# OpenBMB/VisRAG

Measured on NVIDIA H100. Metric: page-images encoded/sec, higher is better.
Workload: dtype bf16

## Files before the change

### visrag_b200/csrc/gemm.cu

```cuda
#include "common.h"
#include "gemm.cuh"

namespace vr {

template <bool F16, int BN, int MODE, bool OUT_F32, bool GELU, bool SWAP = false>
static int launch_gemm(const void* A, int64_t lda, const void* B, int64_t ldb, const GemmArgs& g, cudaStream_t stream) {
    using Cfg = GemmCfg<BN>;
    CUtensorMap ta, tb;
    if (int rc = make_tmap_2d(SWAP ? &tb : &ta, A, g.M, g.K, lda, SWAP ? 64 : GEMM_BM, GEMM_BK, 128, !F16)) return rc;
    if (int rc = make_tmap_2d(SWAP ? &ta : &tb, B, g.N, g.K, ldb, SWAP ? GEMM_BM : 64, GEMM_BK, 128, !F16)) return rc;
    auto kern = gemm_wgmma_kernel<F16, BN, MODE, OUT_F32, GELU, SWAP>;
    static unsigned long long attr_set = 0;
    if (first_use_on_device(&attr_set))
        VR_CHECK_CUDA(cudaFuncSetAttribute(kern, cudaFuncAttributeMaxDynamicSharedMemorySize, Cfg::SMEM_BYTES));
    const int tiles = SWAP ? ((g.N + GEMM_BM - 1) / GEMM_BM) * ((g.M + BN - 1) / BN)
                           : ((g.M + GEMM_BM - 1) / GEMM_BM) * ((g.N + BN - 1) / BN);
    const int grid = tiles < num_sms() ? tiles : num_sms();
    kern<<<grid, GEMM_THREADS, Cfg::SMEM_BYTES, stream>>>(ta, tb, g);
    VR_CHECK_CUDA(cudaGetLastError());
    return 0;
}

template <bool F16, int MODE, bool OUT_F32, bool GELU, int CLUSTER>
static int launch_pingpong(const void* A, int64_t lda, const void* B, int64_t ldb, const GemmArgs& g, bool l2_slices,
                           cudaStream_t stream) {
    CUtensorMap ta, tb;
    if (int rc = make_tmap_2d(&ta, A, g.M, g.K, lda, GEMM_BM, GEMM_BK, 128, !F16)) return rc;
    if (int rc = make_tmap_2d(&tb, B, g.N, g.K, ldb, 64, GEMM_BK, 128, !F16)) return rc;
    auto kern = gemm_pingpong_kernel<F16, MODE, OUT_F32, GELU, CLUSTER>;
    cudaLaunchConfig_t cfg = {};
    cudaLaunchAttribute attr[1];
    cfg.blockDim = dim3(GEMM_THREADS);
    cfg.dynamicSmemBytes = GEMM_PP_SMEM_BYTES;
    cfg.stream = stream;
    attr[0].id = cudaLaunchAttributeClusterDimension;
    attr[0].val.clusterDim.x = CLUSTER;
    attr[0].val.clusterDim.y = 1;
    attr[0].val.clusterDim.z = 1;
    cfg.attrs = attr;
    cfg.numAttrs = 1;
    static unsigned long long attr_set = 0;
    static int max_clusters[64] = {};
    const int dev = current_device(), dev_slot = dev >= 0 && dev < 64 ? dev : 0;
    if (first_use_on_device(&attr_set)) {
        VR_CHECK_CUDA(cudaFuncSetAttribute(kern, cudaFuncAttributeMaxDynamicSharedMemorySize, GEMM_PP_SMEM_BYTES));
        int n = num_sms() / CLUSTER;
        if (CLUSTER > 1) {
            cfg.gridDim = dim3(num_sms() / CLUSTER * CLUSTER);
            VR_CHECK_CUDA(cudaOccupancyMaxActiveClusters(&n, kern, &cfg));
        }
        max_clusters[dev_slot] = n;
    }
    const PPSched sch = pp_schedule(g.M, g.N, g.K, CLUSTER, l2_slices);
    VR_REQUIRE(max_clusters[dev_slot] > 0, "vr_gemm: no %d-CTA cluster of the ping-pong kernel fits on this device", CLUSTER);
    const int units = sch.num_units();
    const int clusters = units < max_clusters[dev_slot] ? units : max_clusters[dev_slot];
    cfg.gridDim = dim3(clusters * CLUSTER);
    VR_CHECK_CUDA(cudaLaunchKernelEx(&cfg, kern, ta, tb, g, sch));
    return 0;
}

template <bool F16>
static int check_out_dtype(const vr_gemm_epilogue& e) {
    if (F16) {
        if (e.mode == VR_EPI_LINEAR && e.out_dtype == VR_F32) {
            VR_REQUIRE(!e.act_gelu, "vr_gemm: GELU epilogue writes fp16 only (fp16 operands)");
            return 0;
        }
        if (e.mode == VR_EPI_LINEAR)
            VR_REQUIRE(e.out_dtype == VR_F16, "vr_gemm: with fp16 operands out_dtype must be VR_F16 or VR_F32");
        else
            VR_REQUIRE(e.out_dtype == VR_F16, "vr_gemm: with fp16 operands ROPE / SWIGLU write fp16: out_dtype must be VR_F16");
        return 0;
    }
    if (e.mode != VR_EPI_LINEAR) return 0;
    if (e.out_dtype == VR_F32) {
        VR_REQUIRE(!e.act_gelu, "vr_gemm: GELU epilogue writes bf16 only");
        return 0;
    }
    VR_REQUIRE(e.out_dtype == VR_BF16, "vr_gemm: out_dtype must be VR_BF16 or VR_F32");
    return 0;
}

template <bool F16>
static int dispatch_swapped(const void* A, int64_t lda, const void* B, int64_t ldb, const GemmArgs& g, cudaStream_t s) {
    const vr_gemm_epilogue& e = g.epi;
    VR_REQUIRE(e.mode == VR_EPI_LINEAR, "vr_gemm: block_n=3 (feature-major accumulator) supports LINEAR epilogues only");
    if (int rc = check_out_dtype<F16>(e)) return rc;
    if (e.out_dtype == VR_F32) return launch_gemm<F16, 128, VR_EPI_LINEAR, true, false, true>(A, lda, B, ldb, g, s);
    if (e.act_gelu) return launch_gemm<F16, 128, VR_EPI_LINEAR, false, true, true>(A, lda, B, ldb, g, s);
    return launch_gemm<F16, 128, VR_EPI_LINEAR, false, false, true>(A, lda, B, ldb, g, s);
}

constexpr int PP = 2, PP_MC = 4, PP_NFAST = 5;
template <bool F16, int BN, int MODE, bool OUT_F32, bool GELU>
static int launch_any(const void* A, int64_t lda, const void* B, int64_t ldb, const GemmArgs& g, cudaStream_t s) {
    if constexpr (BN < 0) return launch_pingpong<F16, MODE, OUT_F32, GELU, -BN == PP_MC ? 2 : 1>(A, lda, B, ldb, g, -BN != PP_NFAST, s);
    else return launch_gemm<F16, BN, MODE, OUT_F32, GELU>(A, lda, B, ldb, g, s);
}

template <bool F16, int BN>
static int dispatch_mode(const void* A, int64_t lda, const void* B, int64_t ldb, const GemmArgs& g, cudaStream_t s) {
    const vr_gemm_epilogue& e = g.epi;
    switch (e.mode) {
        case VR_EPI_LINEAR:
            if (int rc = check_out_dtype<F16>(e)) return rc;
            if (e.out_dtype == VR_F32) return launch_any<F16, BN, VR_EPI_LINEAR, true, false>(A, lda, B, ldb, g, s);
            if (e.act_gelu) return launch_any<F16, BN, VR_EPI_LINEAR, false, true>(A, lda, B, ldb, g, s);
            return launch_any<F16, BN, VR_EPI_LINEAR, false, false>(A, lda, B, ldb, g, s);
        case VR_EPI_ROPE:
            VR_REQUIRE(e.positions && e.rope_cos && e.rope_sin, "vr_gemm: ROPE epilogue needs positions/cos/sin");
            VR_REQUIRE(g.N % 64 == 0 && e.rope_cols % 64 == 0, "vr_gemm: ROPE needs N and rope_cols multiples of 64");
            if (int rc = check_out_dtype<F16>(e)) return rc;
            return launch_any<F16, BN, VR_EPI_ROPE, false, false>(A, lda, B, ldb, g, s);
        case VR_EPI_SWIGLU:
            VR_REQUIRE(g.N % 64 == 0, "vr_gemm: SWIGLU needs N multiple of 64");
            if (int rc = check_out_dtype<F16>(e)) return rc;
            return launch_any<F16, BN, VR_EPI_SWIGLU, false, false>(A, lda, B, ldb, g, s);
        default:
            set_error("vr_gemm: unknown epilogue mode %d", e.mode);
            return 2;
    }
}

template <bool F16>
static int dispatch_block_n(const void* A, int64_t lda, const void* B, int64_t ldb, const GemmArgs& g, int bn, cudaStream_t s) {
    if (bn == PP) return dispatch_mode<F16, -PP>(A, lda, B, ldb, g, s);
    if (bn == PP_MC) return dispatch_mode<F16, -PP_MC>(A, lda, B, ldb, g, s);
    if (bn == PP_NFAST) return dispatch_mode<F16, -PP_NFAST>(A, lda, B, ldb, g, s);
    if (bn == 3) return dispatch_swapped<F16>(A, lda, B, ldb, g, s);
    if (bn == 256) return dispatch_mode<F16, 256>(A, lda, B, ldb, g, s);
    if (bn == 192) return dispatch_mode<F16, 192>(A, lda, B, ldb, g, s);
    if (bn == 128) return dispatch_mode<F16, 128>(A, lda, B, ldb, g, s);
    if (bn == 64) return dispatch_mode<F16, 64>(A, lda, B, ldb, g, s);
    set_error("vr_gemm: block_n must be 0 (auto), 64, 128, 192, 256, 2 / 4 / 5 (ping-pong) or 3 (feature-major accumulator)");
    return 2;
}

}

extern "C" int vr_gemm_tuned(const void* A, int64_t lda, const void* B, int64_t ldb, int32_t ab_dtype, int32_t M,
                             int32_t N, int32_t K, const vr_gemm_epilogue* epi, int32_t block_n, void* stream) {
    using namespace vr;
    VR_REQUIRE(A && B && epi && epi->out, "vr_gemm: null pointer argument");
    VR_REQUIRE(M > 0 && N > 0 && K > 0, "vr_gemm: empty problem M=%d N=%d K=%d", M, N, K);
    VR_REQUIRE(ab_dtype == VR_BF16 || ab_dtype == VR_F16, "vr_gemm: operands must be bf16 or fp16 (got dtype %d)", ab_dtype);
    VR_REQUIRE(N % 8 == 0, "vr_gemm: N=%d must be a multiple of 8", N);
    VR_REQUIRE(K % 8 == 0, "vr_gemm: K=%d must be a multiple of 8 (16-byte TMA rows)", K);
    const int64_t out_cols = epi->mode == VR_EPI_SWIGLU ? N / 2 : N;
    VR_REQUIRE(epi->ldo >= out_cols && epi->ldo % 8 == 0, "vr_gemm: ldo=%lld too small or not a multiple of 8",
               (long long)epi->ldo);
    GemmArgs g;
    g.M = M; g.N = N; g.K = K; g.epi = *epi;
    cudaStream_t s = reinterpret_cast<cudaStream_t>(stream);
    int bn = block_n;
    if (bn == 0) {
        bn = M <= 128 ? 64 : PP_MC;
    }
    return ab_dtype == VR_F16 ? dispatch_block_n<true>(A, lda, B, ldb, g, bn, s) : dispatch_block_n<false>(A, lda, B, ldb, g, bn, s);
}

extern "C" int vr_gemm(const void* A, int64_t lda, const void* B, int64_t ldb, int32_t ab_dtype, int32_t M, int32_t N,
                       int32_t K, const vr_gemm_epilogue* epi, void* stream) {
    return vr_gemm_tuned(A, lda, B, ldb, ab_dtype, M, N, K, epi, 0, stream);
}
```

### visrag_b200/csrc/gemm.cuh

```cuda
#pragma once
#include "ptx.cuh"
#include "../../include/visrag_b200.h"

namespace vr {

constexpr int GEMM_BM = 128;
constexpr int GEMM_BK = 64;
constexpr int GEMM_THREADS = 3 * 128;

template <int BN>
struct GemmCfg {
    static_assert(BN % 64 == 0 && BN <= 256, "tile width: 64, 128, 192 or 256");
    static constexpr int A_BYTES = GEMM_BM * GEMM_BK * 2;
    static constexpr int B_BYTES = BN * GEMM_BK * 2;
    static constexpr int STAGE_BYTES = A_BYTES + B_BYTES;
    static constexpr int STAGES = (192 * 1024) / STAGE_BYTES;
    static constexpr int SMEM_BYTES = STAGES * STAGE_BYTES + 1024  + 256 ;
};

struct GemmArgs {
    int M, N, K;
    vr_gemm_epilogue epi;
};

__device__ __forceinline__ float erf_as(float x) {
    const float ax = fabsf(x);
    float t;
    asm("rcp.approx.ftz.f32 %0, %1;" : "=f"(t) : "f"(fmaf(0.3275911f, ax, 1.0f)));
    float p = fmaf(1.061405429f, t, -1.453152027f);
    p = fmaf(p, t, 1.421413741f);
    p = fmaf(p, t, -0.284496736f);
    p = fmaf(p, t, 0.254829592f);
    p *= t;
    float e;
    asm("ex2.approx.ftz.f32 %0, %1;" : "=f"(e) : "f"(-1.4426950408889634f * ax * ax));
    return copysignf(fmaf(-p, e, 1.0f), x);
}
__device__ __forceinline__ float gelu_erf(float x) { return 0.5f * x * (1.0f + erf_as(x * 0.70710678118654752f)); }

__device__ __forceinline__ void pk_fma(float& d0, float& d1, float a0, float a1, float b0, float b1, float c0, float c1) {
    d0 = fmaf(a0, b0, c0);
    d1 = fmaf(a1, b1, c1);
}
#ifndef VR_GELU_POLY
#define VR_GELU_POLY 1
#endif
#if VR_GELU_POLY
__device__ __forceinline__ void gelu_erf2(float& x0, float& x1) {
    constexpr float R2 = 0.70710678118654752f, ZMAX = 3.2f, A = 2.0f / (ZMAX * ZMAX);
    const float z0 = fminf(fmaxf(x0 * R2, -ZMAX), ZMAX), z1 = fminf(fmaxf(x1 * R2, -ZMAX), ZMAX);
    float w0, w1, u0, u1, p0, p1;
    pk_fma(w0, w1, z0, z1, z0, z1, 0.0f, 0.0f);
    pk_fma(u0, u1, w0, w1, A, A, -1.0f, -1.0f);
    pk_fma(p0, p1, u0, u1, 2.982273671e-03f, 2.982273671e-03f, -7.046153472e-03f, -7.046153472e-03f);
    pk_fma(p0, p1, p0, p1, u0, u1, 7.957076705e-03f, 7.957076705e-03f);
    pk_fma(p0, p1, p0, p1, u0, u1, -1.521942819e-02f, -1.521942819e-02f);
    pk_fma(p0, p1, p0, p1, u0, u1, 3.318292224e-02f, 3.318292224e-02f);
    pk_fma(p0, p1, p0, p1, u0, u1, -5.471928813e-02f, -5.471928813e-02f);
    pk_fma(p0, p1, p0, p1, u0, u1, 8.062700147e-02f, 8.062700147e-02f);
    pk_fma(p0, p1, p0, p1, u0, u1, -1.136467381e-01f, -1.136467381e-01f);
    pk_fma(p0, p1, p0, p1, u0, u1, 1.543549678e-01f, 1.543549678e-01f);
    pk_fma(p0, p1, p0, p1, u0, u1, -2.173077339e-01f, -2.173077339e-01f);
    pk_fma(p0, p1, p0, p1, u0, u1, 4.413341836e-01f, 4.413341836e-01f);
    float r0, r1;
    pk_fma(r0, r1, p0, p1, z0, z1, 0.0f, 0.0f);
    const float h0 = 0.5f * x0, h1 = 0.5f * x1;
    pk_fma(x0, x1, h0, h1, r0, r1, h0, h1);
}
#else
__device__ __forceinline__ void gelu_erf2(float& x0, float& x1) {
    constexpr float R2 = 0.70710678118654752f;
    const float a0 = fabsf(x0) * R2, a1 = fabsf(x1) * R2;
    float d0, d1, t0, t1, p0, p1, q0, q1, e0, e1, r0, r1;
    pk_fma(d0, d1, a0, a1, 0.3275911f, 0.3275911f, 1.0f, 1.0f);
    asm("rcp.approx.ftz.f32 %0, %1;" : "=f"(t0) : "f"(d0));
    asm("rcp.approx.ftz.f32 %0, %1;" : "=f"(t1) : "f"(d1));
    pk_fma(p0, p1, t0, t1, 1.061405429f, 1.061405429f, -1.453152027f, -1.453152027f);
    pk_fma(p0, p1, p0, p1, t0, t1, 1.421413741f, 1.421413741f);
    pk_fma(p0, p1, p0, p1, t0, t1, -0.284496736f, -0.284496736f);
    pk_fma(p0, p1, p0, p1, t0, t1, 0.254829592f, 0.254829592f);
    pk_fma(p0, p1, p0, p1, t0, t1, 0.0f, 0.0f);
    pk_fma(q0, q1, a0, a1, a0, a1, 0.0f, 0.0f);
    asm("ex2.approx.ftz.f32 %0, %1;" : "=f"(e0) : "f"(q0 * -1.4426950408889634f));
    asm("ex2.approx.ftz.f32 %0, %1;" : "=f"(e1) : "f"(q1 * -1.4426950408889634f));
    pk_fma(r0, r1, p0, p1, -e0, -e1, 1.0f, 1.0f);
    r0 = copysignf(r0, x0);
    r1 = copysignf(r1, x1);
    const float h0 = 0.5f * x0, h1 = 0.5f * x1;
    pk_fma(x0, x1, h0, h1, r0, r1, h0, h1);
}
#endif
__device__ __forceinline__ float silu(float x) {
    float e, r;
    asm("ex2.approx.ftz.f32 %0, %1;" : "=f"(e) : "f"(x * -1.4426950408889634f));
    asm("rcp.approx.ftz.f32 %0, %1;" : "=f"(r) : "f"(1.0f + e));
    return x * r;
}

template <bool F16, bool OUT_F32, bool GELU>
__device__ __forceinline__ void epi_linear2(const GemmArgs& g, int row, int col, float x0, float x1) {
    const vr_gemm_epilogue& e = g.epi;
    if (row >= g.M || col >= g.N) return;
    if (e.bias) {
        const float2 b = *reinterpret_cast<const float2*>(e.bias + col);
        x0 += b.x; x1 += b.y;
    }
    if (GELU) gelu_erf2(x0, x1);
    if (e.scale != 1.0f) { x0 *= e.scale; x1 *= e.scale; }
    if (e.rowadd) {
        const float2 a2 = *reinterpret_cast<const float2*>(e.rowadd + static_cast<long long>(row % e.rowadd_period) * g.N + col);
        x0 += a2.x; x1 += a2.y;
    }
    const long long o = static_cast<long long>(row) * e.ldo + col;
    if (e.resid) {
        const float2 r2 = *reinterpret_cast<const float2*>(e.resid + o);
        x0 += r2.x; x1 += r2.y;
    }
    if (OUT_F32) *reinterpret_cast<float2*>(reinterpret_cast<float*>(e.out) + o) = make_float2(x0, x1);
    else *reinterpret_cast<uint32_t*>(reinterpret_cast<half16_t<F16>*>(e.out) + o) = pack16x2<F16>(x0, x1);
}

template <bool F16, bool OUT_F32, bool GELU>
__device__ __forceinline__ void epi_linear_t(const GemmArgs& g, int tok, int f, float x) {
    const vr_gemm_epilogue& e = g.epi;
    if (tok >= g.M || f >= g.N) return;
    if (e.bias) x += e.bias[f];
    if (GELU) {
        float y = x;
        gelu_erf2(x, y);
    }
    if (e.scale != 1.0f) x *= e.scale;
    if (e.rowadd) x += e.rowadd[static_cast<long long>(tok % e.rowadd_period) * g.N + f];
    const long long o = static_cast<long long>(tok) * e.ldo + f;
    if (e.resid) x += e.resid[o];
    if (OUT_F32) reinterpret_cast<float*>(e.out)[o] = x;
    else reinterpret_cast<half16_t<F16>*>(e.out)[o] = to_half16<F16>(x);
}

template <bool F16>
__device__ __forceinline__ void epi_rope2(const GemmArgs& g, int row, int head0, int c, float lo0, float lo1, float hi0,
                                          float hi1) {
    const vr_gemm_epilogue& e = g.epi;
    if (row >= g.M || head0 >= g.N) return;
    if (head0 < e.rope_cols) {
        const long long pos = e.positions[row];
        const float2 cs = *reinterpret_cast<const float2*>(e.rope_cos + pos * 32 + c);
        const float2 sn = *reinterpret_cast<const float2*>(e.rope_sin + pos * 32 + c);
        const float a0 = lo0, a1 = lo1, b0 = hi0, b1 = hi1;
        lo0 = a0 * cs.x - b0 * sn.x; hi0 = b0 * cs.x + a0 * sn.x;
        lo1 = a1 * cs.y - b1 * sn.y; hi1 = b1 * cs.y + a1 * sn.y;
    }
    half16_t<F16>* o = reinterpret_cast<half16_t<F16>*>(e.out) + static_cast<long long>(row) * e.ldo + head0 + c;
    *reinterpret_cast<uint32_t*>(o) = pack16x2<F16>(lo0, lo1);
    *reinterpret_cast<uint32_t*>(o + 32) = pack16x2<F16>(hi0, hi1);
}

template <bool F16>
__device__ __forceinline__ void epi_swiglu2(const GemmArgs& g, int row, int blk0, int c, float g0, float g1, float u0, float u1) {
    const vr_gemm_epilogue& e = g.epi;
    if (row >= g.M || blk0 >= g.N) return;
    half16_t<F16>* o = reinterpret_cast<half16_t<F16>*>(e.out) + static_cast<long long>(row) * e.ldo + (blk0 >> 1) + c;
    *reinterpret_cast<uint32_t*>(o) = pack16x2<F16>(silu(g0) * u0, silu(g1) * u1);
}

template <bool F16, int BN, int MODE, bool OUT_F32, bool GELU, bool SWAP = false>
__global__ void __launch_bounds__(GEMM_THREADS, 1)
gemm_wgmma_kernel(const __grid_constant__ CUtensorMap tmap_a, const __grid_constant__ CUtensorMap tmap_b, const GemmArgs g) {
    using Cfg = GemmCfg<BN>;
    constexpr int STAGES = Cfg::STAGES;

    extern __shared__ uint8_t smem_raw[];
    uint8_t* smem = reinterpret_cast<uint8_t*>((reinterpret_cast<uintptr_t>(smem_raw) + 1023) & ~uintptr_t(1023));
    uint8_t* smem_a = smem;
    uint8_t* smem_b = smem + STAGES * Cfg::A_BYTES;
    uint64_t* full_bar = reinterpret_cast<uint64_t*>(smem + STAGES * Cfg::STAGE_BYTES);
    uint64_t* empty_bar = full_bar + STAGES;

    const int wg = threadIdx.x >> 7;
    const int warp = (threadIdx.x >> 5) & 3;
    const int lane = threadIdx.x & 31;

    static_assert(!SWAP || MODE == VR_EPI_LINEAR, "feature-major accumulators are implemented for LINEAR epilogues");
    const int tiles_m = ((SWAP ? g.N : g.M) + GEMM_BM - 1) / GEMM_BM;
    const int tiles_n = ((SWAP ? g.M : g.N) + BN - 1) / BN;
    const int num_tiles = tiles_m * tiles_n;
    const int num_kb = (g.K + GEMM_BK - 1) / GEMM_BK;
    auto tile_m0 = [&](int t) { return (SWAP ? t % tiles_m : t / tiles_n) * GEMM_BM; };
    auto tile_n0 = [&](int t) { return (SWAP ? t / tiles_m : t % tiles_n) * BN; };

    if (threadIdx.x == 0) {
        tma_prefetch_desc(&tmap_a);
        tma_prefetch_desc(&tmap_b);
        for (int i = 0; i < STAGES; ++i) {
            mbar_init(&full_bar[i], 1);
            mbar_init(&empty_bar[i], 8);
        }
        fence_mbar_init();
    }
    __syncthreads();

    if (wg == 0) {
        setmaxnreg_dec<40>();
        if (warp == 0 && lane == 0) {
            int stage = 0;
            uint32_t phase = 0;
            for (int t = blockIdx.x; t < num_tiles; t += gridDim.x) {
                const int m0 = tile_m0(t);
                const int n0 = tile_n0(t);
                for (int kb = 0; kb < num_kb; ++kb) {
                    mbar_wait(&empty_bar[stage], phase ^ 1);
                    mbar_expect_tx(&full_bar[stage], Cfg::STAGE_BYTES);
                    tma_load_2d(&tmap_a, &full_bar[stage], smem_a + stage * Cfg::A_BYTES, kb * GEMM_BK, m0);
#pragma unroll
                    for (int h = 0; h < BN / 64; ++h)
                        tma_load_2d(&tmap_b, &full_bar[stage], smem_b + stage * Cfg::B_BYTES + h * (64 * GEMM_BK * 2),
                                    kb * GEMM_BK, n0 + h * 64);
                    if (++stage == STAGES) { stage = 0; phase ^= 1; }
                }
            }
        }
    } else {
        setmaxnreg_inc<232>();
        const int cw = wg - 1;
        const uint64_t desc_hi = make_smem_desc(0, 16, 1024, kLayoutSW128);
        const uint32_t a_lo0 = (smem_u32(smem_a) + cw * (64 * GEMM_BK * 2)) >> 4, b_lo0 = smem_u32(smem_b) >> 4;
        const int g8 = lane >> 2, q = lane & 3;
        int stage = 0;
        uint32_t phase = 0;
        for (int t = blockIdx.x; t < num_tiles; t += gridDim.x) {
            float acc[BN / 2];
            int prev = -1;
            for (int kb = 0; kb < num_kb; ++kb) {
                mbar_wait(&full_bar[stage], phase);
                const uint64_t ad = desc_hi | static_cast<uint64_t>(a_lo0 + stage * (Cfg::A_BYTES >> 4));
                const uint64_t bd = desc_hi | static_cast<uint64_t>(b_lo0 + stage * (Cfg::B_BYTES >> 4));
                wgmma_fence();
#pragma unroll
                for (int kk = 0; kk < 4; ++kk)
                    wgmma_ss<F16, false>(acc, ad + 2 * kk, bd + 2 * kk, (kb | kk) != 0, std::integral_constant<int, BN>());
                wgmma_commit();
                if (prev >= 0) {
                    wgmma_wait<1>();
                    if (lane == 0) mbar_arrive(&empty_bar[prev]);
                }
                prev = stage;
                if (++stage == STAGES) { stage = 0; phase ^= 1; }
            }
            wgmma_wait<0>();
            if (lane == 0) mbar_arrive(&empty_bar[prev]);
            wgmma_touch(acc);

            const int r0 = tile_m0(t) + cw * 64 + warp * 16 + g8;
            const int n0 = tile_n0(t);
            if (MODE == VR_EPI_LINEAR) {
#pragma unroll
                for (int j = 0; j < BN / 8; ++j) {
                    const int c = n0 + j * 8 + q * 2;
                    if (SWAP) {
                        epi_linear_t<F16, OUT_F32, GELU>(g, c, r0, acc[4 * j]);
                        epi_linear_t<F16, OUT_F32, GELU>(g, c + 1, r0, acc[4 * j + 1]);
                        epi_linear_t<F16, OUT_F32, GELU>(g, c, r0 + 8, acc[4 * j + 2]);
                        epi_linear_t<F16, OUT_F32, GELU>(g, c + 1, r0 + 8, acc[4 * j + 3]);
                    } else {
                        epi_linear2<F16, OUT_F32, GELU>(g, r0, c, acc[4 * j], acc[4 * j + 1]);
                        epi_linear2<F16, OUT_F32, GELU>(g, r0 + 8, c, acc[4 * j + 2], acc[4 * j + 3]);
                    }
                }
            } else {
#pragma unroll
                for (int hb = 0; hb < BN / 64; ++hb) {
#pragma unroll
                    for (int j = 0; j < 4; ++j) {
                        const int lo = 4 * (hb * 8 + j), hi = 4 * (hb * 8 + j + 4);
                        const int blk0 = n0 + hb * 64, c = j * 8 + q * 2;
                        if (MODE == VR_EPI_ROPE) {
                            epi_rope2<F16>(g, r0, blk0, c, acc[lo], acc[lo + 1], acc[hi], acc[hi + 1]);
                            epi_rope2<F16>(g, r0 + 8, blk0, c, acc[lo + 2], acc[lo + 3], acc[hi + 2], acc[hi + 3]);
                        } else {
                            epi_swiglu2<F16>(g, r0, blk0, c, acc[lo], acc[lo + 1], acc[hi], acc[hi + 1]);
                            epi_swiglu2<F16>(g, r0 + 8, blk0, c, acc[lo + 2], acc[lo + 3], acc[hi + 2], acc[hi + 3]);
                        }
                    }
                }
            }
        }
    }
}

constexpr int GEMM_PP_BN = 128;
constexpr int GEMM_PP_A_BYTES = GEMM_BM * GEMM_BK * 2;
constexpr int GEMM_PP_B_BYTES = GEMM_PP_BN * GEMM_BK * 2;
constexpr int GEMM_PP_STAGE_BYTES = GEMM_PP_A_BYTES + GEMM_PP_B_BYTES;
constexpr int GEMM_PP_STAGES = (192 * 1024) / GEMM_PP_STAGE_BYTES;
constexpr int GEMM_PP_SMEM_BYTES = GEMM_PP_STAGES * GEMM_PP_STAGE_BYTES + 1024 + 256;
constexpr int GEMM_PP_BAR_TURN = 1;

constexpr long long GEMM_PP_L2_SLICE = 20ll << 20;

struct PPSched {
    int units_m, tiles_n, slice_w;
    __host__ __device__ int num_units() const { return units_m * tiles_n; }
    __device__ void coords(int u, int& um, int& tn) const {
        const int slice_units = units_m * slice_w;
        const int s = u / slice_units, r = u - s * slice_units;
        const int w = min(slice_w, tiles_n - s * slice_w);
        um = r / w;
        tn = s * slice_w + r % w;
    }
};

inline PPSched pp_schedule(int M, int N, int K, int cluster, bool l2_slices) {
    PPSched s;
    s.units_m = ((M + GEMM_BM - 1) / GEMM_BM + cluster - 1) / cluster;
    s.tiles_n = (N + GEMM_PP_BN - 1) / GEMM_PP_BN;
    s.slice_w = s.tiles_n;
    if (l2_slices) {
        long long fit = GEMM_PP_L2_SLICE / (static_cast<long long>(GEMM_PP_BN) * K * 2);
        if (fit < 1) fit = 1;
        if (fit < s.tiles_n) {
            const int slices = static_cast<int>((s.tiles_n + fit - 1) / fit);
            s.slice_w = (s.tiles_n + slices - 1) / slices;
        }
    }
    return s;
}

constexpr int PP_EPI_BATCH = 4;
template <bool F16, bool OUT_F32, bool GELU>
__device__ __forceinline__ void pp_epilogue_linear(const GemmArgs& g, const float (&acc)[64], int r0, int n0, int q2) {
    const vr_gemm_epilogue& e = g.epi;
    const bool row_ok[2] = {r0 < g.M, r0 + 8 < g.M};
    const long long o[2] = {static_cast<long long>(r0) * e.ldo, static_cast<long long>(r0 + 8) * e.ldo};
    long long ra[2] = {0, 0};
    if (e.rowadd) {
        ra[0] = static_cast<long long>(r0 % e.rowadd_period) * g.N;
        ra[1] = static_cast<long long>((r0 + 8) % e.rowadd_period) * g.N;
    }
#pragma unroll
    for (int jb = 0; jb < GEMM_PP_BN / 8; jb += PP_EPI_BATCH) {
        float2 bias[PP_EPI_BATCH], add[PP_EPI_BATCH][2], res[PP_EPI_BATCH][2];
#pragma unroll
        for (int j = 0; j < PP_EPI_BATCH; ++j) {
            const int c = n0 + (jb + j) * 8 + q2;
            const bool col_ok = c < g.N;
            bias[j] = make_float2(0.0f, 0.0f);
            if (e.bias && col_ok) bias[j] = __ldg(reinterpret_cast<const float2*>(e.bias + c));
#pragma unroll
            for (int h = 0; h < 2; ++h) {
                add[j][h] = res[j][h] = make_float2(0.0f, 0.0f);
                if (e.rowadd && col_ok && row_ok[h]) add[j][h] = __ldg(reinterpret_cast<const float2*>(e.rowadd + ra[h] + c));
                if (e.resid && col_ok && row_ok[h]) res[j][h] = *reinterpret_cast<const float2*>(e.resid + o[h] + c);
            }
        }
#pragma unroll
        for (int j = 0; j < PP_EPI_BATCH; ++j) {
            const int c = n0 + (jb + j) * 8 + q2;
#pragma unroll
            for (int h = 0; h < 2; ++h) {
                if (!row_ok[h] || c >= g.N) continue;
                float x0 = acc[4 * (jb + j) + 2 * h], x1 = acc[4 * (jb + j) + 2 * h + 1];
                if (e.bias) { x0 += bias[j].x; x1 += bias[j].y; }
                if (GELU) gelu_erf2(x0, x1);
                if (e.scale != 1.0f) { x0 *= e.scale; x1 *= e.scale; }
                if (e.rowadd) { x0 += add[j][h].x; x1 += add[j][h].y; }
                if (e.resid) { x0 += res[j][h].x; x1 += res[j][h].y; }
                if (OUT_F32) *reinterpret_cast<float2*>(reinterpret_cast<float*>(e.out) + o[h] + c) = make_float2(x0, x1);
                else *reinterpret_cast<uint32_t*>(reinterpret_cast<half16_t<F16>*>(e.out) + o[h] + c) = pack16x2<F16>(x0, x1);
            }
        }
    }
}

template <bool F16, int MODE, bool OUT_F32, bool GELU>
__device__ __forceinline__ void pp_epilogue(const GemmArgs& g, const float (&acc)[64], int r0, int n0, int q2) {
    if (MODE == VR_EPI_LINEAR) {
        pp_epilogue_linear<F16, OUT_F32, GELU>(g, acc, r0, n0, q2);
    } else {
#pragma unroll
        for (int hb = 0; hb < GEMM_PP_BN / 64; ++hb) {
#pragma unroll
            for (int j = 0; j < 4; ++j) {
                const int lo = 4 * (hb * 8 + j), hi = 4 * (hb * 8 + j + 4);
                const int blk0 = n0 + hb * 64, c = j * 8 + q2;
                if (MODE == VR_EPI_ROPE) {
                    epi_rope2<F16>(g, r0, blk0, c, acc[lo], acc[lo + 1], acc[hi], acc[hi + 1]);
                    epi_rope2<F16>(g, r0 + 8, blk0, c, acc[lo + 2], acc[lo + 3], acc[hi + 2], acc[hi + 3]);
                } else {
                    epi_swiglu2<F16>(g, r0, blk0, c, acc[lo], acc[lo + 1], acc[hi], acc[hi + 1]);
                    epi_swiglu2<F16>(g, r0 + 8, blk0, c, acc[lo + 2], acc[lo + 3], acc[hi + 2], acc[hi + 3]);
                }
            }
        }
    }
}

template <bool F16, int MODE, bool OUT_F32, bool GELU, int CLUSTER>
__global__ void __launch_bounds__(GEMM_THREADS, 1)
gemm_pingpong_kernel(const __grid_constant__ CUtensorMap tmap_a, const __grid_constant__ CUtensorMap tmap_b, const GemmArgs g,
                     const PPSched sch) {
    static_assert(CLUSTER == 1 || CLUSTER == 2, "CTA pairs at most");
    constexpr int STAGES = GEMM_PP_STAGES;
    extern __shared__ uint8_t smem_raw[];
    uint8_t* smem = reinterpret_cast<uint8_t*>((reinterpret_cast<uintptr_t>(smem_raw) + 1023) & ~uintptr_t(1023));
    uint8_t* smem_a = smem;
    uint8_t* smem_b = smem + STAGES * GEMM_PP_A_BYTES;
    uint64_t* full_bar = reinterpret_cast<uint64_t*>(smem + STAGES * GEMM_PP_STAGE_BYTES);
    uint64_t* empty_bar = full_bar + STAGES;

    const int wg = threadIdx.x >> 7;
    const int warp = (threadIdx.x >> 5) & 3;
    const int lane = threadIdx.x & 31;
    const int num_kb = (g.K + GEMM_BK - 1) / GEMM_BK;
    const int rank = CLUSTER == 1 ? 0 : static_cast<int>(cluster_ctarank());
    const int unit0 = blockIdx.x / CLUSTER, unit_step = gridDim.x / CLUSTER;
    const int num_units = sch.num_units();

    if (threadIdx.x == 0) {
        tma_prefetch_desc(&tmap_a);
        tma_prefetch_desc(&tmap_b);
        for (int i = 0; i < STAGES; ++i) {
            mbar_init(&full_bar[i], 1);
            mbar_init(&empty_bar[i], 4 * CLUSTER);
        }
        fence_mbar_init();
    }
    if (CLUSTER == 1) __syncthreads();
    else cluster_sync_all();

    if (wg == 0) {
        setmaxnreg_dec<40>();
        if (warp == 0 && lane == 0) {
            int stage = 0;
            uint32_t phase = 0;
            for (int u = unit0; u < num_units; u += unit_step) {
                int um, tn;
                sch.coords(u, um, tn);
                const int m0 = (um * CLUSTER + rank) * GEMM_BM, n0 = tn * GEMM_PP_BN;
                for (int kb = 0; kb < num_kb; ++kb) {
                    mbar_wait(&empty_bar[stage], phase ^ 1);
                    mbar_expect_tx(&full_bar[stage], GEMM_PP_STAGE_BYTES);
                    tma_load_2d(&tmap_a, &full_bar[stage], smem_a + stage * GEMM_PP_A_BYTES, kb * GEMM_BK, m0);
                    uint8_t* b_dst = smem_b + stage * GEMM_PP_B_BYTES;
                    if (CLUSTER == 1) {
#pragma unroll
                        for (int h = 0; h < GEMM_PP_BN / 64; ++h)
                            tma_load_2d(&tmap_b, &full_bar[stage], b_dst + h * (64 * GEMM_BK * 2), kb * GEMM_BK, n0 + h * 64);
                    } else {
                        tma_load_2d_multicast(&tmap_b, &full_bar[stage], b_dst + rank * (64 * GEMM_BK * 2), kb * GEMM_BK,
                                              n0 + rank * 64, 0x3);
                    }
                    if (++stage == STAGES) { stage = 0; phase ^= 1; }
                }
            }
        }
    } else {
        setmaxnreg_inc<232>();
        const int me = wg - 1;
        const uint64_t desc_hi = make_smem_desc(0, 16, 1024, kLayoutSW128);
        const uint32_t a_lo0 = smem_u32(smem_a) >> 4, b_lo0 = smem_u32(smem_b) >> 4;
        constexpr uint32_t HALF = (64 * GEMM_BK * 2) >> 4;
        const int g8 = lane >> 2, q = lane & 3;
        auto release = [&](int s) {
            if (lane != 0) return;
            if (CLUSTER == 1) {
                mbar_arrive(&empty_bar[s]);
            } else {
#pragma unroll
                for (int r = 0; r < CLUSTER; ++r) mbar_arrive_cluster(&empty_bar[s], r);
            }
        };
        for (int i = me, u = unit0 + me * unit_step; u < num_units; i += 2, u += 2 * unit_step) {
            const int pos = i * num_kb;
            int stage = pos % STAGES;
            uint32_t phase = (pos / STAGES) & 1;
            if (i > 0) named_bar_sync(GEMM_PP_BAR_TURN + me, 256);
            float acc0[64], acc1[64];
            int prev = -1;
            for (int kb = 0; kb < num_kb; ++kb) {
                mbar_wait(&full_bar[stage], phase);
                const uint64_t ad = desc_hi | static_cast<uint64_t>(a_lo0 + stage * (GEMM_PP_A_BYTES >> 4));
                const uint64_t bd = desc_hi | static_cast<uint64_t>(b_lo0 + stage * (GEMM_PP_B_BYTES >> 4));
                wgmma_fence();
#pragma unroll
                for (int kk = 0; kk < 4; ++kk) {
                    wgmma_ss<F16, false>(acc0, ad + 2 * kk, bd + 2 * kk, (kb | kk) != 0, std::integral_constant<int, 128>());
                    wgmma_ss<F16, false>(acc1, ad + HALF + 2 * kk, bd + 2 * kk, (kb | kk) != 0,
                                           std::integral_constant<int, 128>());
                }
                wgmma_commit();
                if (prev >= 0) {
                    wgmma_wait<1>();
                    release(prev);
                }
                prev = stage;
                if (++stage == STAGES) { stage = 0; phase ^= 1; }
            }
            if (u + unit_step < num_units) named_bar_arrive(GEMM_PP_BAR_TURN + (me ^ 1), 256);
            wgmma_wait<0>();
            release(prev);
            wgmma_touch(acc0);
            wgmma_touch(acc1);

            int um, tn;
            sch.coords(u, um, tn);
            const int m0 = (um * CLUSTER + rank) * GEMM_BM, n0 = tn * GEMM_PP_BN;
            pp_epilogue<F16, MODE, OUT_F32, GELU>(g, acc0, m0 + warp * 16 + g8, n0, q * 2);
            pp_epilogue<F16, MODE, OUT_F32, GELU>(g, acc1, m0 + 64 + warp * 16 + g8, n0, q * 2);
        }
    }
    if (CLUSTER == 2) cluster_sync_all();
}

}
```

### visrag_b200/encoder.py

```python
from __future__ import annotations

import functools
import os
from collections import OrderedDict
from typing import Dict, Optional, Sequence, Tuple

import numpy as np
import torch

from . import _lib as L
from . import ops
from .config import VisRAGConfig
from .host import PreparedBatch, prepare_batch
from .weights import sincos_2d

VIT_HEAD_STRIDE = 80

GRAPH_MAX_VIT_TOKENS = 32 * 1024
GRAPH_MAX_LM_TOKENS = 4096
GRAPH_TEXT_BUCKET = 16
GRAPH_CACHE = 12


class _GraphEntry:
    __slots__ = ("graph", "groups", "src", "pos", "cu", "reps", "launches")


def _half(t: torch.Tensor, dev, dtype: torch.dtype) -> torch.Tensor:
    return t.to(device=dev, dtype=dtype).contiguous()


def _f32(t: torch.Tensor, dev) -> torch.Tensor:
    return t.to(device=dev, dtype=torch.float32).contiguous()


def _on_own_device(fn):

    @functools.wraps(fn)
    def wrapper(self, *args, **kwargs):
        with L.on_device(self.device):
            return fn(self, *args, **kwargs)

    return wrapper


class VisRAGEngine:

    def __init__(self, cfg: VisRAGConfig, state_dict: Dict[str, torch.Tensor], device: str = "cuda:0",
                 max_vit_tokens: int = 131072, device_frontend: bool = True, cuda_graphs: Optional[bool] = None,
                 dtype: torch.dtype = torch.bfloat16):
        cfg.validate()
        if dtype not in ops.HALF_DTYPES:
            raise ValueError(f"VisRAGEngine: dtype must be torch.bfloat16 or torch.float16, got {dtype}")
        L.lib()
        self.cfg = cfg
        self.dtype = dtype
        self.device_frontend = device_frontend
        self.device = L.norm_device(device)
        self.max_vit_tokens = max_vit_tokens
        self.cuda_graphs = (os.environ.get("VR_CUDA_GRAPHS", "1") != "0") if cuda_graphs is None else bool(cuda_graphs)
        self._graphs: "OrderedDict[tuple, _GraphEntry]" = OrderedDict()
        self._graph_seen: Dict[tuple, int] = {}
        self.graph_stats = {"captured": 0, "replayed": 0, "eager": 0}
        with L.on_device(self.device):
            self._load(cfg, state_dict)

    def _load(self, cfg: VisRAGConfig, state_dict: Dict[str, torch.Tensor]) -> None:
        sd, dev, dt = state_dict, self.device, self.dtype
        D, E, H, I = cfg.vit_dim, cfg.hidden, cfg.hidden, cfg.inter
        nh, hd, hs = cfg.vit_heads, cfg.vit_head_dim, VIT_HEAD_STRIDE
        with torch.no_grad():
            P2 = 3 * cfg.patch_size ** 2
            self.patch_k = ((P2 + 63) // 64) * 64
            pw = sd["vpm.patch_embed.proj.weight"].float().reshape(D, P2)
            w = torch.zeros((D, self.patch_k), dtype=torch.float32, device=pw.device)
            w[:, :P2] = pw
            self.patch_w = _half(w, dev, dt)
            self.patch_b = _f32(sd["vpm.patch_embed.proj.bias"], dev)
            self.pos_embed = sd["vpm.pos_embed"].float().cpu()
            self._pos_cache: Dict[Tuple[int, int], torch.Tensor] = {}
            self._sincos_cache: Dict[Tuple[int, int], torch.Tensor] = {}
            self.blocks = []
            for i in range(cfg.vit_depth):
                p = f"vpm.blocks.{i}."
                wq = sd[p + "attn.qkv.weight"].float().reshape(3, nh, hd, D)
                bq = sd[p + "attn.qkv.bias"].float().reshape(3, nh, hd)
                wpad = torch.zeros((3, nh, hs, D), device=wq.device)
                bpad = torch.zeros((3, nh, hs), device=wq.device)
                wpad[:, :, :hd] = wq
                bpad[:, :, :hd] = bq
                self.blocks.append(dict(
                    n1w=_f32(sd[p + "norm1.weight"], dev), n1b=_f32(sd[p + "norm1.bias"], dev),
                    qkv_w=_half(wpad.reshape(3 * nh * hs, D), dev, dt), qkv_b=_f32(bpad.reshape(-1), dev),
                    proj_w=_half(sd[p + "attn.proj.weight"], dev, dt), proj_b=_f32(sd[p + "attn.proj.bias"], dev),
                    n2w=_f32(sd[p + "norm2.weight"], dev), n2b=_f32(sd[p + "norm2.bias"], dev),
                    fc1_w=_half(sd[p + "mlp.fc1.weight"], dev, dt), fc1_b=_f32(sd[p + "mlp.fc1.bias"], dev),
                    fc2_w=_half(sd[p + "mlp.fc2.weight"], dev, dt), fc2_b=_f32(sd[p + "mlp.fc2.bias"], dev),
                ))
            self.vnorm_w, self.vnorm_b = _f32(sd["vpm.norm.weight"], dev), _f32(sd["vpm.norm.bias"], dev)
            self.rs_kv_w = _half(sd["resampler.kv_proj.weight"], dev, dt)
            self.rs_lnkv = (_f32(sd["resampler.ln_kv.weight"], dev), _f32(sd["resampler.ln_kv.bias"], dev))
            self.rs_lnpost = (_f32(sd["resampler.ln_post.weight"], dev), _f32(sd["resampler.ln_post.bias"], dev))
            Win, bin_ = sd["resampler.attn.in_proj_weight"].float(), sd["resampler.attn.in_proj_bias"].float()
            self.rs_wk, self.rs_bk = _half(Win[E:2 * E], dev, dt), _f32(bin_[E:2 * E], dev)
            self.rs_wv, self.rs_bv = _half(Win[2 * E:], dev, dt), _f32(bin_[2 * E:], dev)
            self.rs_wo, self.rs_bo = _half(sd["resampler.attn.out_proj.weight"], dev, dt), _f32(sd["resampler.attn.out_proj.bias"], dev)
            self.rs_projT = _half(sd["resampler.proj"].float().t(), dev, dt)
            q_in = ops.layernorm(_f32(sd["resampler.query"], dev), _f32(sd["resampler.ln_q.weight"], dev),
                                 _f32(sd["resampler.ln_q.bias"], dev), 1e-6, add=_f32(sd["resampler.pos_embed"], dev), dtype=dt)[1]
            self.rs_q = torch.zeros((128, E), dtype=dt, device=dev)
            ops.gemm(q_in, _half(Win[:E], dev, dt), bias=_f32(bin_[:E], dev), out=self.rs_q[: cfg.query_num])
            self.embed = _half(sd["llm.model.embed_tokens.weight"], dev, dt)
            self.layers = []
            for i in range(cfg.layers):
                p = f"llm.model.layers.{i}."
                wqkv = torch.cat([sd[p + f"self_attn.{n}_proj.weight"].float() for n in ("q", "k", "v")], dim=0)
                wg, wu = sd[p + "mlp.gate_proj.weight"].float(), sd[p + "mlp.up_proj.weight"].float()
                wgu = torch.stack([wg.reshape(I // 32, 32, H), wu.reshape(I // 32, 32, H)], dim=1).reshape(2 * I, H)
                self.layers.append(dict(
                    in_w=_f32(sd[p + "input_layernorm.weight"], dev), post_w=_f32(sd[p + "post_attention_layernorm.weight"], dev),
                    qkv_w=_half(wqkv, dev, dt), o_w=_half(sd[p + "self_attn.o_proj.weight"], dev, dt),
                    gu_w=_half(wgu, dev, dt), down_w=_half(sd[p + "mlp.down_proj.weight"], dev, dt),
                ))
            self.final_w = _f32(sd["llm.model.norm.weight"], dev)
            inv = 1.0 / (cfg.rope_theta ** (torch.arange(0, cfg.head_dim, 2).float() / cfg.head_dim))
            fr = torch.outer(torch.arange(cfg.max_pos).float(), inv)
            self.rope_cos, self.rope_sin = _f32(fr.cos(), dev), _f32(fr.sin(), dev)
            torch.cuda.synchronize(dev)

    def _pos_table(self, gh: int, gw: int) -> torch.Tensor:
        key = (gh, gw)
        if key not in self._pos_cache:
            S, D = self.cfg.vit_pos_grid, self.cfg.vit_dim
            if gh == S and gw == S:
                t = self.pos_embed[0]
            else:
                p = self.pos_embed.reshape(1, S, S, D).permute(0, 3, 1, 2)
                p = torch.nn.functional.interpolate(p, size=(gh, gw), mode="bicubic", antialias=True)
                t = p.permute(0, 2, 3, 1).reshape(gh * gw, D)
            self._pos_cache[key] = _f32(t, self.device)
        return self._pos_cache[key]

    def _sincos_table(self, gh: int, gw: int) -> torch.Tensor:
        key = (gh, gw)
        if key not in self._sincos_cache:
            self._sincos_cache[key] = _f32(torch.from_numpy(sincos_2d(self.cfg.hidden, gh, gw)), self.device)
        return self._sincos_cache[key]

    @_on_own_device
    def vit_tokens(self, pixels: torch.Tensor) -> torch.Tensor:
        cfg, dt = self.cfg, self.dtype
        S, h, w, _ = pixels.shape
        gh, gw = h // cfg.patch_size, w // cfg.patch_size
        N, D, nh = gh * gw, cfg.vit_dim, cfg.vit_heads
        M = S * N
        a = ops.im2col_norm(pixels, cfg.patch_size, self.patch_k, dt)
        x = ops.gemm(a, self.patch_w, bias=self.patch_b, rowadd=self._pos_table(gh, gw), out_dtype=torch.float32)
        cu = torch.arange(0, (S + 1) * N, N, dtype=torch.int32, device=self.device)
        qkv = torch.empty((M, 3 * nh * VIT_HEAD_STRIDE), dtype=dt, device=self.device)
        att = torch.empty((M, D), dtype=dt, device=self.device)
        scale = cfg.vit_head_dim ** -0.5
        for blk in self.blocks:
            y = ops.layernorm(x, blk["n1w"], blk["n1b"], cfg.ln_eps, dtype=dt)
            ops.gemm(y, blk["qkv_w"], bias=blk["qkv_b"], out=qkv)
            ops.attention(qkv, qkv, qkv, q_col0=0, k_col0=nh * VIT_HEAD_STRIDE, v_col0=2 * nh * VIT_HEAD_STRIDE,
                          head_stride=VIT_HEAD_STRIDE, head_dim=cfg.vit_head_dim, heads=nh, batch=S, cu_k=cu, max_k=N,
                          cu_q=cu, max_q=N, causal=False, scale=scale, out=att)
            ops.gemm(att, blk["proj_w"], bias=blk["proj_b"], resid=x, out=x, out_dtype=torch.float32)
            y = ops.layernorm(x, blk["n2w"], blk["n2b"], cfg.ln_eps, dtype=dt)
            y = ops.gemm(y, blk["fc1_w"], bias=blk["fc1_b"], gelu=True)
            ops.gemm(y, blk["fc2_w"], bias=blk["fc2_b"], resid=x, out=x, out_dtype=torch.float32)
        return ops.layernorm(x, self.vnorm_w, self.vnorm_b, cfg.ln_eps, dtype=dt)

    @_on_own_device
    def resample(self, tokens: torch.Tensor, S: int, gh: int, gw: int, out: torch.Tensor) -> None:
        cfg, dt = self.cfg, self.dtype
        E, N, nh = cfg.hidden, gh * gw, cfg.rs_heads
        kv = ops.gemm(tokens, self.rs_kv_w, out_dtype=torch.float32)
        v_in, k_in = ops.layernorm(kv, self.rs_lnkv[0], self.rs_lnkv[1], 1e-6, add=self._sincos_table(gh, gw), dtype=dt)
        k = ops.gemm(k_in, self.rs_wk, bias=self.rs_bk)
        v = ops.gemm(v_in, self.rs_wv, bias=self.rs_bv)
        cu = torch.arange(0, (S + 1) * N, N, dtype=torch.int32, device=self.device)
        att = torch.empty((S * cfg.query_num, E), dtype=dt, device=self.device)
        ops.attention(self.rs_q, k, v, q_col0=0, k_col0=0, v_col0=0, head_stride=128, head_dim=128, heads=nh, batch=S,
                      cu_k=cu, max_k=N, cu_q=None, max_q=cfg.query_num, causal=False, scale=128 ** -0.5, out=att)
        o = ops.gemm(att, self.rs_wo, bias=self.rs_bo, out_dtype=torch.float32)
        o = ops.layernorm(o, self.rs_lnpost[0], self.rs_lnpost[1], 1e-6, dtype=dt)
        ops.gemm(o, self.rs_projT, out=out, out_dtype=torch.float32)

    @_on_own_device
    def encode_vision(self, groups: Dict[Tuple[int, int], torch.Tensor], group_row0: Dict[Tuple[int, int], int],
                      n_slices: int) -> Optional[torch.Tensor]:
        if n_slices == 0:
            return None
        cfg = self.cfg
        out = torch.empty((n_slices * cfg.query_num, cfg.hidden), dtype=torch.float32, device=self.device)
        for (h, w), px in groups.items():
            gh, gw = h // cfg.patch_size, w // cfg.patch_size
            per = max(1, self.max_vit_tokens // (gh * gw))
            for s0 in range(0, px.shape[0], per):
                chunk = px[s0:s0 + per]
                S = chunk.shape[0]
                r0 = (group_row0[(h, w)] + s0) * cfg.query_num
                self.resample(self.vit_tokens(chunk), S, gh, gw, out[r0:r0 + S * cfg.query_num])
        return out

    @_on_own_device
    def lm_hidden(self, token_src: torch.Tensor, positions: torch.Tensor, cu: torch.Tensor, max_len: int,
                  vision: Optional[torch.Tensor]) -> torch.Tensor:
        cfg, dt = self.cfg, self.dtype
        H, nh = cfg.hidden, cfg.heads
        B = cu.shape[0] - 1
        h = ops.build_lm_input(token_src, self.embed, cfg.scale_emb, vision)
        T = h.shape[0]
        qkv = torch.empty((T, 3 * H), dtype=dt, device=self.device)
        att = torch.empty((T, H), dtype=dt, device=self.device)
        s = cfg.depth_scale
        for lyr in self.layers:
            a = ops.rmsnorm(h, lyr["in_w"], cfg.rms_eps, dt)
            ops.gemm(a, lyr["qkv_w"], mode=L.VR_EPI_ROPE, positions=positions, rope_cos=self.rope_cos,
                     rope_sin=self.rope_sin, rope_cols=2 * H, out=qkv)
            ops.attention(qkv, qkv, qkv, q_col0=0, k_col0=H, v_col0=2 * H, head_stride=64, head_dim=64, heads=nh, batch=B,
                          cu_k=cu, max_k=max_len, cu_q=cu, max_q=max_len, causal=True, scale=cfg.head_dim ** -0.5, out=att)
            ops.gemm(att, lyr["o_w"], resid=h, out=h, scale=s, out_dtype=torch.float32)
            a = ops.rmsnorm(h, lyr["post_w"], cfg.rms_eps, dt)
            a = ops.gemm(a, lyr["gu_w"], mode=L.VR_EPI_SWIGLU)
            ops.gemm(a, lyr["down_w"], resid=h, out=h, scale=s, out_dtype=torch.float32)
        return h

    def _pinned_buf(self, key, n: int, dtype) -> torch.Tensor:
        buf = self._pinned.get(key)
        if buf is None or buf.numel() < n or buf.dtype != dtype:
            buf = torch.empty(max(n, 1), dtype=dtype).pin_memory()
            self._pinned[key] = buf
        return buf[:n]

    def _stage(self, a: np.ndarray, key) -> torch.Tensor:
        t = torch.from_numpy(np.ascontiguousarray(a))
        stage = self._pinned_buf(key, t.numel(), t.dtype).view(t.shape)
        stage.copy_(t)
        return stage.to(self.device, non_blocking=True)

    def _stage_slices(self, slices, key) -> torch.Tensor:
        h, w, c = slices[0].shape
        stage = self._pinned_buf(key, len(slices) * h * w * c, torch.uint8).view(len(slices), h, w, c)
        dst = stage.numpy()
        for j, a in enumerate(slices):
            dst[j] = a
        return stage.to(self.device, non_blocking=True)

    def _upload_group(self, key, slices, s: int) -> torch.Tensor:
        host = [i for i, a in enumerate(slices) if a is not None]
        if len(host) == len(slices):
            return self._stage_slices(slices, (s, "px", key))
        dev = torch.empty((len(slices), key[0], key[1], 3), dtype=torch.uint8, device=self.device)
        if host:
            dev[torch.tensor(host, device=self.device)] = self._stage_slices([slices[i] for i in host], (s, "px", key))
        return dev

    def _render_jobs(self, jobs, groups, s: int) -> None:
        from .frontend import DeviceFrontEnd

        if not hasattr(self, "_frontend"):
            self._frontend = DeviceFrontEnd(self.device)
        by_size = {}
        for j in jobs:
            by_size.setdefault(j.pixels.shape, []).append(j)
        for (H, W, ps), lst in by_size.items():
            pages = self._stage_slices([j.pixels for j in lst], (s, "page", (H, W, ps)))
            plan = lst[0].plan
            tkey = lst[0].thumb[0]
            first = self._stage(np.asarray([j.thumb[1] for j in lst], dtype=np.int32), (s, "first_t", (H, W, ps)))
            self._frontend.resize_into(pages, plan.source_size[0], plan.source_size[1], groups[tkey], first,
                                       plan.source_size[0], plan.source_size[1])
            if plan.grid is not None:
                ckey = lst[0].cells[0]
                first = self._stage(np.asarray([j.cells[1] for j in lst], dtype=np.int32), (s, "first_c", (H, W, ps)))
                self._frontend.resize_into(pages, plan.refine_size[0], plan.refine_size[1], groups[ckey], first,
                                           plan.cell_size[0], plan.cell_size[1])
            pages.record_stream(torch.cuda.current_stream(self.device))

    @_on_own_device
    def upload(self, pb: PreparedBatch):
        if not hasattr(self, "_pinned"):
            self._pinned, self._upload_done, self._flip = {}, [None, None], 0
            self._copy_stream = torch.cuda.Stream(device=self.device)
        s = self._flip
        self._flip ^= 1
        if self._upload_done[s] is not None:
            self._upload_done[s].synchronize()
        compute = torch.cuda.current_stream(self.device)
        with torch.cuda.stream(self._copy_stream):
            groups = {k: self._upload_group(k, v, s) for k, v in pb.groups.items()}
            if pb.jobs:
                self._render_jobs(pb.jobs, groups, s)
            out = (groups, self._stage(pb.token_src, (s, "src")), self._stage(pb.positions, (s, "pos")),
                   self._stage(pb.cu_seqlens, (s, "cu")))
            ev = torch.cuda.Event()
            ev.record()
        self._upload_done[s] = ev
        compute.wait_event(ev)
        for t in (*groups.values(), *out[1:]):
            t.record_stream(compute)
        return out

    @_on_own_device
    def encode_device(self, groups, group_row0, n_slices: int, src, pos, cu, max_len: int, pooling: str = "wmean",
                      normalize: bool = True, return_hidden: bool = False):
        vision = self.encode_vision(groups, group_row0, n_slices)
        h = self.lm_hidden(src, pos, cu, max_len, vision)
        reps = ops.pool_norm(h, self.final_w, self.cfg.rms_eps, cu, pooling, normalize)
        return (reps, h) if return_hidden else reps

    def _graph_plan(self, pb: PreparedBatch):
        if not self.cuda_graphs or pb.n_items == 0:
            return None
        T = int(pb.cu_seqlens[-1])
        max_len = int(pb.seq_lens.max())
        vit_tokens = sum(len(v) * (k[0] // self.cfg.patch_size) * (k[1] // self.cfg.patch_size) for k, v in pb.groups.items())
        if vit_tokens > GRAPH_MAX_VIT_TOKENS or T > GRAPH_MAX_LM_TOKENS:
            return None
        if pb.n_slices > 0:
            return pb.token_src, pb.positions, pb.cu_seqlens, max_len, pb.n_items
        b = GRAPH_TEXT_BUCKET
        Tb = -(-(T + 1) // b) * b
        pad = Tb - T
        Lb = min(-(-max(max_len, pad) // b) * b, self.cfg.max_pos)
        if pad > self.cfg.max_pos:
            return None
        src = np.concatenate([pb.token_src, np.full(pad, -1, dtype=np.int32)])
        pos = np.concatenate([pb.positions, np.arange(pad, dtype=np.int32)])
        cu = np.concatenate([pb.cu_seqlens, np.asarray([Tb], dtype=np.int32)])
        return src, pos, cu, Lb, pb.n_items

    def _encode_graphed(self, sig, groups, group_row0, n_slices, src, pos, cu, max_len, pooling, normalize):
        ent = self._graphs.get(sig)
        if ent is None:
            seen = self._graph_seen.get(sig, 0)
            if len(self._graph_seen) > 4096:
                self._graph_seen.clear()
            self._graph_seen[sig] = seen + 1
            if seen == 0:
                self.graph_stats["eager"] += 1
                return self.encode_device(groups, group_row0, n_slices, src, pos, cu, max_len, pooling, normalize)
            if seen < 0:
                self.graph_stats["eager"] += 1
                return self.encode_device(groups, group_row0, n_slices, src, pos, cu, max_len, pooling, normalize)
            ent = _GraphEntry()
            ent.groups = {k: v.clone() for k, v in groups.items()}
            ent.src, ent.pos, ent.cu = src.clone(), pos.clone(), cu.clone()
            launches0 = L.LAUNCHES
            torch.cuda.synchronize(self.device)
            ent.graph = torch.cuda.CUDAGraph()
            try:
                with torch.cuda.graph(ent.graph):
                    ent.reps = self.encode_device(ent.groups, group_row0, n_slices, ent.src, ent.pos, ent.cu, max_len, pooling, normalize)
            except Exception as exc:
                import warnings

                warnings.warn(f"visrag_b200: CUDA-graph capture failed for this batch shape ({exc!r}); using eager launches")
                self._graph_seen[sig] = -(1 << 30)
                self.graph_stats["eager"] += 1
                return self.encode_device(groups, group_row0, n_slices, src, pos, cu, max_len, pooling, normalize)
            ent.launches = L.LAUNCHES - launches0
            self._graphs[sig] = ent
            self.graph_stats["captured"] += 1
            while len(self._graphs) > GRAPH_CACHE:
                self._graphs.popitem(last=False)
        else:
            self._graphs.move_to_end(sig)
            for k, v in groups.items():
                ent.groups[k].copy_(v, non_blocking=True)
            ent.src.copy_(src, non_blocking=True)
            ent.pos.copy_(pos, non_blocking=True)
            ent.cu.copy_(cu, non_blocking=True)
        ent.graph.replay()
        L.LAUNCHES += ent.launches
        self.graph_stats["replayed"] += 1
        return ent.reps.clone()

    @_on_own_device
    def encode_prepared(self, pb: PreparedBatch, pooling: str = "wmean", normalize: bool = True,
                        return_hidden: bool = False):
        if pb.n_items == 0:
            return torch.zeros((0, self.cfg.hidden), dtype=torch.float32, device=self.device)
        if int(pb.seq_lens.max()) > self.cfg.max_pos:
            raise ValueError(f"sequence longer than max_pos={self.cfg.max_pos}")
        plan = None if return_hidden or ops.profiling() else self._graph_plan(pb)
        if plan is not None:
            src_h, pos_h, cu_h, max_len, n_out = plan
            shaped = PreparedBatch(pb.n_items, pb.seq_lens, cu_h, pos_h, src_h, pb.groups, pb.group_row0, pb.n_slices, pb.jobs)
            groups, src, pos, cu = self.upload(shaped)
            sig = (tuple(sorted((k, v.shape[0]) for k, v in groups.items())), tuple(sorted(pb.group_row0.items())), pb.n_slices,
                   int(src.shape[0]), int(cu.shape[0]), max_len, pooling, bool(normalize))
            reps = self._encode_graphed(sig, groups, pb.group_row0, pb.n_slices, src, pos, cu, max_len, pooling, normalize)
            return reps[:n_out]
        groups, src, pos, cu = self.upload(pb)
        return self.encode_device(groups, pb.group_row0, pb.n_slices, src, pos, cu, int(pb.seq_lens.max()), pooling,
                                  normalize, return_hidden)

    @_on_own_device
    def encode(self, texts: Sequence[str], images: Sequence, tokenizer, max_inp_length: Optional[int] = 2048,
               pooling: str = "wmean", normalize: bool = True) -> torch.Tensor:
        pb = prepare_batch(texts, images, tokenizer, self.cfg, max_inp_length, self.device_frontend)
        return self.encode_prepared(pb, pooling, normalize)
```

Before: 303.0.

## Write 16-byte epilogue stores via quad shuffle transpose and pad ViT MLP width

The ping-pong GEMM linear epilogue for half outputs now gathers four column groups per quad using warp shuffles, so each thread writes one 16-byte vector instead of four 4-byte stores. To keep those stores aligned, the ViT MLP intermediate width is zero-padded to a multiple of 64 in the fc1 weights and bias and the fc2 input columns. A new check requires LINEAR outputs to be 16-byte aligned. In exchange the epilogue runs extra shuffles, and the padded MLP does a little extra GEMM work.

```diff
diff --git a/visrag_b200/csrc/gemm.cu b/visrag_b200/csrc/gemm.cu
--- a/visrag_b200/csrc/gemm.cu
+++ b/visrag_b200/csrc/gemm.cu
@@ -150,6 +150,8 @@
     const int64_t out_cols = epi->mode == VR_EPI_SWIGLU ? N / 2 : N;
     VR_REQUIRE(epi->ldo >= out_cols && epi->ldo % 8 == 0, "vr_gemm: ldo=%lld too small or not a multiple of 8",
                (long long)epi->ldo);
+    VR_REQUIRE(epi->mode != VR_EPI_LINEAR || (reinterpret_cast<uintptr_t>(epi->out) & 15) == 0,
+               "vr_gemm: a LINEAR out must be 16-byte aligned (out=%p)", epi->out);
     GemmArgs g;
     g.M = M; g.N = N; g.K = K; g.epi = *epi;
     cudaStream_t s = reinterpret_cast<cudaStream_t>(stream);
diff --git a/visrag_b200/csrc/gemm.cuh b/visrag_b200/csrc/gemm.cuh
--- a/visrag_b200/csrc/gemm.cuh
+++ b/visrag_b200/csrc/gemm.cuh
@@ -325,6 +325,16 @@
     return s;
 }
 
+__device__ __forceinline__ void quad_transpose4(uint32_t (&w)[4], int q) {
+    const bool b1 = q & 2, b0 = q & 1;
+    uint32_t r0 = __shfl_xor_sync(0xffffffffu, b1 ? w[0] : w[2], 2);
+    uint32_t r1 = __shfl_xor_sync(0xffffffffu, b1 ? w[1] : w[3], 2);
+    if (b1) { w[0] = r0; w[1] = r1; } else { w[2] = r0; w[3] = r1; }
+    r0 = __shfl_xor_sync(0xffffffffu, b0 ? w[0] : w[1], 1);
+    r1 = __shfl_xor_sync(0xffffffffu, b0 ? w[2] : w[3], 1);
+    if (b0) { w[0] = r0; w[2] = r1; } else { w[1] = r0; w[3] = r1; }
+}
+
 constexpr int PP_EPI_BATCH = 4;
 template <bool F16, bool OUT_F32, bool GELU>
 __device__ __forceinline__ void pp_epilogue_linear(const GemmArgs& g, const float (&acc)[64], int r0, int n0, int q2) {
@@ -352,12 +362,13 @@
                 if (e.resid && col_ok && row_ok[h]) res[j][h] = *reinterpret_cast<const float2*>(e.resid + o[h] + c);
             }
         }
+        uint32_t w16[2][PP_EPI_BATCH];
 #pragma unroll
         for (int j = 0; j < PP_EPI_BATCH; ++j) {
             const int c = n0 + (jb + j) * 8 + q2;
 #pragma unroll
             for (int h = 0; h < 2; ++h) {
-                if (!row_ok[h] || c >= g.N) continue;
+                if (OUT_F32 && (!row_ok[h] || c >= g.N)) continue;
                 float x0 = acc[4 * (jb + j) + 2 * h], x1 = acc[4 * (jb + j) + 2 * h + 1];
                 if (e.bias) { x0 += bias[j].x; x1 += bias[j].y; }
                 if (GELU) gelu_erf2(x0, x1);
@@ -365,7 +376,18 @@
                 if (e.rowadd) { x0 += add[j][h].x; x1 += add[j][h].y; }
                 if (e.resid) { x0 += res[j][h].x; x1 += res[j][h].y; }
                 if (OUT_F32) *reinterpret_cast<float2*>(reinterpret_cast<float*>(e.out) + o[h] + c) = make_float2(x0, x1);
-                else *reinterpret_cast<uint32_t*>(reinterpret_cast<half16_t<F16>*>(e.out) + o[h] + c) = pack16x2<F16>(x0, x1);
+                else w16[h][j] = pack16x2<F16>(x0, x1);
+            }
+        }
+        if (!OUT_F32) {
+            static_assert(PP_EPI_BATCH == 4, "the quad transpose moves 4 column groups");
+            const int q = q2 >> 1, c = n0 + (jb + q) * 8;
+#pragma unroll
+            for (int h = 0; h < 2; ++h) {
+                quad_transpose4(w16[h], q);
+                if (row_ok[h] && c < g.N)
+                    *reinterpret_cast<uint4*>(reinterpret_cast<half16_t<F16>*>(e.out) + o[h] + c) =
+                        make_uint4(w16[h][0], w16[h][1], w16[h][2], w16[h][3]);
             }
         }
     }
diff --git a/visrag_b200/encoder.py b/visrag_b200/encoder.py
--- a/visrag_b200/encoder.py
+++ b/visrag_b200/encoder.py
@@ -7,6 +7,7 @@
 
 import numpy as np
 import torch
+import torch.nn.functional as F
 
 from . import _lib as L
 from . import ops
@@ -15,6 +16,7 @@
 from .weights import sincos_2d
 
 VIT_HEAD_STRIDE = 80
+VIT_MLP_ALIGN = 64
 
 GRAPH_MAX_VIT_TOKENS = 32 * 1024
 GRAPH_MAX_LM_TOKENS = 4096
@@ -81,6 +83,8 @@
             self._pos_cache: Dict[Tuple[int, int], torch.Tensor] = {}
             self._sincos_cache: Dict[Tuple[int, int], torch.Tensor] = {}
             self.blocks = []
+            mlp = cfg.vit_mlp
+            mlp_pad = -(-mlp // VIT_MLP_ALIGN) * VIT_MLP_ALIGN - mlp
             for i in range(cfg.vit_depth):
                 p = f"vpm.blocks.{i}."
                 wq = sd[p + "attn.qkv.weight"].float().reshape(3, nh, hd, D)
@@ -94,8 +98,9 @@
                     qkv_w=_half(wpad.reshape(3 * nh * hs, D), dev, dt), qkv_b=_f32(bpad.reshape(-1), dev),
                     proj_w=_half(sd[p + "attn.proj.weight"], dev, dt), proj_b=_f32(sd[p + "attn.proj.bias"], dev),
                     n2w=_f32(sd[p + "norm2.weight"], dev), n2b=_f32(sd[p + "norm2.bias"], dev),
-                    fc1_w=_half(sd[p + "mlp.fc1.weight"], dev, dt), fc1_b=_f32(sd[p + "mlp.fc1.bias"], dev),
-                    fc2_w=_half(sd[p + "mlp.fc2.weight"], dev, dt), fc2_b=_f32(sd[p + "mlp.fc2.bias"], dev),
+                    fc1_w=_half(F.pad(sd[p + "mlp.fc1.weight"], (0, 0, 0, mlp_pad)), dev, dt),
+                    fc1_b=_f32(F.pad(sd[p + "mlp.fc1.bias"], (0, mlp_pad)), dev),
+                    fc2_w=_half(F.pad(sd[p + "mlp.fc2.weight"], (0, mlp_pad)), dev, dt), fc2_b=_f32(sd[p + "mlp.fc2.bias"], dev),
                 ))
             self.vnorm_w, self.vnorm_b = _f32(sd["vpm.norm.weight"], dev), _f32(sd["vpm.norm.bias"], dev)
             self.rs_kv_w = _half(sd["resampler.kv_proj.weight"], dev, dt)
```

Measured after the change: 323.6 (median of 6 runs). +6.8%, better.
